# f-dangel/vivit

Hardware: AMD Instinct MI355X
Metric: GGN eigenpairs/sec (Gram build + symeig), MLP 784-512-10, batch=4096 (higher is better)
Workload: dtype f32

## Files before the change

### vivit_amd/csrc/sy2sb.hip

```cpp
#include <cstdlib>

#include "common.h"
#include "device_utils.h"
#include "eig_internal.h"

namespace vivit {

constexpr int SNB = 64;
constexpr int QT = 128;
constexpr int SGRP = 8;

__global__ __launch_bounds__(256) void sb_panel_load_kernel(const float *__restrict__ A, int64_t lda, int64_t j0, int64_t mp,
                                                            float *__restrict__ pan) {
  const int64_t idx = (int64_t)blockIdx.x * 256 + threadIdx.x;
  if (idx >= mp * SNB) return;
  const int64_t r = idx / SNB, c = idx - r * SNB;
  pan[idx] = A[(j0 + SNB + r) * lda + j0 + c];
}

__global__ __launch_bounds__(256) void sb_panel_load_row_kernel(const float *__restrict__ A, int64_t lda, int64_t j0, int64_t mp,
                                                                float *__restrict__ pan) {
  __shared__ float t[SNB][SNB + 1];
  const int64_t r0 = (int64_t)blockIdx.x * SNB;
  const int tid = threadIdx.x;
  for (int idx = tid; idx < SNB * SNB; idx += 256) {
    const int c = idx / SNB, rr = idx % SNB;
    t[c][rr] = r0 + rr < mp ? A[(j0 + c) * lda + j0 + SNB + r0 + rr] : 0.f;
  }
  __syncthreads();
  for (int idx = tid; idx < SNB * SNB; idx += 256) {
    const int rr = idx / SNB, c = idx % SNB;
    if (r0 + rr < mp) pan[(r0 + rr) * SNB + c] = t[c][rr];
  }
}

__global__ __launch_bounds__(256) void coef_gather_kernel(const float *__restrict__ S, int64_t lds_, int64_t g, int kp,
                                                          float *__restrict__ Coef) {
  const int idx = blockIdx.x * 256 + threadIdx.x;
  if (idx >= SNB * kp) return;
  const int k = idx / SNB, m = idx % SNB;
  Coef[(int64_t)m * kp + k] = S[(int64_t)k * lds_ + g + m];
}


__global__ __launch_bounds__(256) void qr_step_kernel(float *__restrict__ pan, int64_t mp, int c, int ncol, int nwg, QrPart pt,
                                                      float *__restrict__ vdst1, float *__restrict__ vdst2, int64_t lds_, int64_t gi0,
                                                      float *__restrict__ A, int64_t lda, int64_t j0,
                                                      float *__restrict__ tau1, float *__restrict__ betas) {
  __shared__ float tile[QT][SNB + 1];
  __shared__ float vs[QT], xs2[QT];
  __shared__ float zs[SNB];
  __shared__ float zq[4][SNB];
  __shared__ __attribute__((aligned(16))) float zq16[16][SNB];
  const int tid = threadIdx.x;
  const int64_t r0 = (int64_t)blockIdx.x * QT;
  constexpr int NTL = QT * (SNB / 4) / 256;
  float4 tl[NTL];
#pragma unroll
  for (int i = 0; i < NTL; ++i) {
    const int idx = tid + 256 * i;
    const int rl = idx / (SNB / 4), c4 = (idx - rl * (SNB / 4)) * 4;
    const int64_t r = r0 + rl;
    tl[i] = *reinterpret_cast<const float4 *>(pan + (r < mp ? r : 0) * SNB + c4);
  }
  const int par = c & 1;
  const float *uin = pt.u + (int64_t)par * nwg * SNB;
  const float *din = pt.diag + par * SNB;
  const int cq4 = tid & 15, q16 = tid >> 4;
  float4 pv[20];
#pragma unroll
  for (int i = 0; i < 20; ++i) {
    const int w = q16 + 16 * i;
    pv[i] = *reinterpret_cast<const float4 *>(uin + (int64_t)(w < nwg ? w : 0) * SNB + 4 * cq4);
  }
  const float din_c = din[c >= 0 ? c : 0], din_t = din[tid & (SNB - 1)];
  __builtin_amdgcn_sched_barrier(0);
#pragma unroll
  for (int i = 0; i < NTL; ++i) {
    const int idx = tid + 256 * i;
    const int rl = idx / (SNB / 4), c4 = (idx - rl * (SNB / 4)) * 4;
    const bool ok = r0 + rl < mp;
    tile[rl][c4 + 0] = ok ? tl[i].x : 0.f;
    tile[rl][c4 + 1] = ok ? tl[i].y : 0.f;
    tile[rl][c4 + 2] = ok ? tl[i].z : 0.f;
    tile[rl][c4 + 3] = ok ? tl[i].w : 0.f;
  }
  if (c >= 0) {
    {
      float4 acc = make_float4(0.f, 0.f, 0.f, 0.f);
#pragma unroll
      for (int i = 0; i < 20; ++i)
        if (q16 + 16 * i < nwg) { acc.x += pv[i].x; acc.y += pv[i].y; acc.z += pv[i].z; acc.w += pv[i].w; }
      for (int w0 = q16 + 16 * 20; w0 < nwg; w0 += 16 * 20) {
        float4 v[20];
#pragma unroll
        for (int i = 0; i < 20; ++i) {
          const int w = w0 + 16 * i;
          v[i] = *reinterpret_cast<const float4 *>(uin + (int64_t)(w < nwg ? w : 0) * SNB + 4 * cq4);
        }
#pragma unroll
        for (int i = 0; i < 20; ++i)
          if (w0 + 16 * i < nwg) { acc.x += v[i].x; acc.y += v[i].y; acc.z += v[i].z; acc.w += v[i].w; }
      }
      *reinterpret_cast<float4 *>(&zq16[q16][4 * cq4]) = acc;
    }
    __syncthreads();
    float ssq = 0.f;
#pragma unroll
    for (int g2 = 0; g2 < 16; ++g2) ssq += zq16[g2][c];
    const float alpha = din_c;
    float tau = 0.f, beta = alpha, scal = 0.f;
    if (ssq > 0.f) {
      beta = -copysignf(sqrt_nr(alpha * alpha + ssq), alpha);
      tau = (beta - alpha) * rcp_nr(beta);
      scal = rcp_nr(alpha - beta);
    }
    if (tid < SNB) {
      float u = 0.f;
#pragma unroll
      for (int g2 = 0; g2 < 16; ++g2) u += zq16[g2][tid];
      zs[tid] = tid > c ? tau * (din_t + scal * u) : 0.f;
    }
    if (tid < QT) {
      const int64_t r = r0 + tid;
      float v = 0.f;
      if (r < mp) {
        if (r == c) v = 1.f;
        else if (r > c) v = tile[tid][c] * scal;
        vdst1[(int64_t)c * lds_ + gi0 + r] = v;
        vdst2[(int64_t)c * lds_ + gi0 + r] = v;
        if (r >= c) A[(j0 + c) * lda + gi0 + r] = v;
      }
      vs[tid] = v;
    }
    if (blockIdx.x == 0 && tid == 0) { tau1[j0 + c] = tau; betas[c] = beta; }
  } else {
    if (tid < QT) vs[tid] = 0.f;
    if (tid < SNB) zs[tid] = 0.f;
  }
  __syncthreads();
  const int cn = c + 1;
  const bool has_next = cn < ncol;
  if (tid < QT) {
    const int64_t r = r0 + tid;
    xs2[tid] = (has_next && r > cn && r < mp) ? tile[tid][cn] - vs[tid] * zs[cn] : 0.f;
  }
  __syncthreads();
  {
    const int cc = tid & 63, q = tid >> 6;
    const float zc = zs[cc];
    float acc = 0.f;
#pragma unroll 8
    for (int i = 0; i < QT / 4; ++i) {
      const int rl = q + 4 * i;
      const float v = vs[rl];
      float x = tile[rl][cc];
      if (cc > c && v != 0.f) {
        x -= v * zc;
        tile[rl][cc] = x;
        if (r0 + rl < mp) pan[(r0 + rl) * SNB + cc] = x;
      }
      acc += xs2[rl] * x;
    }
    zq[q][cc] = acc;
  }
  if (!has_next) return;
  __syncthreads();
  {
    const int par = cn & 1;
    if (tid < SNB) pt.u[((int64_t)par * nwg + blockIdx.x) * SNB + tid] = (zq[0][tid] + zq[1][tid]) + (zq[2][tid] + zq[3][tid]);
    if (cn >= r0 && cn < r0 + QT && tid < SNB) pt.diag[par * SNB + tid] = tile[cn - r0][tid];
  }
}

constexpr int QP_WG = 32, QP_THREADS = 512;
struct QrPersistWs {
  float *ubuf;
  float *dbuf;
  int *counter;
  int *tmo;
  int attempt;
  int fault;
};

__device__ __forceinline__ float sel8(float a0, float a1, float a2, float a3, float a4, float a5, float a6, float a7, int j) {
  const float t0 = (j & 1) ? a1 : a0, t1 = (j & 1) ? a3 : a2, t2 = (j & 1) ? a5 : a4, t3 = (j & 1) ? a7 : a6;
  const float u0 = (j & 2) ? t1 : t0, u1 = (j & 2) ? t3 : t2;
  return (j & 4) ? u1 : u0;
}

template <int RI>
__global__ __launch_bounds__(QP_THREADS) void qr_persist_kernel(float *__restrict__ pan, int64_t mp, int ncol, QrPersistWs pw,
                                                                float *__restrict__ vdst1, float *__restrict__ vdst2, int64_t lds_,
                                                                int64_t gi0, float *__restrict__ A, int64_t lda, int64_t j0,
                                                                float *__restrict__ tau1, float *__restrict__ betas) {
  if ((blockIdx.x & 7) != 0) return;
  if (pw.attempt == 1 && __hip_atomic_load(pw.counter + 1, __ATOMIC_RELAXED, __HIP_MEMORY_SCOPE_AGENT) != PERSIST_ABORT) return;
  int *const cnt = pw.counter + 8 * pw.attempt;
  const int w = blockIdx.x >> 3;
  const int tid = threadIdx.x, lane = tid & 63, wave = tid >> 6;
  const int cg = tid & 7, rs = tid >> 3;
  constexpr int RW = 64 * RI;
  const int64_t rbase = (int64_t)w * RW;
  __shared__ float s_u[SNB], s_d[SNB], s_dn[SNB];
  __shared__ float s_red[QP_THREADS / 64][SNB];
  __shared__ float s_v[RW];
  __shared__ int s_flag[2];

  float x[RI][8];
#pragma unroll
  for (int i = 0; i < RI; ++i) {
    const int64_t r = rbase + rs + 64 * i;
    const float *src = pan + (r < mp ? r : 0) * SNB + 8 * cg;
    const float4 a = *reinterpret_cast<const float4 *>(src), b = *reinterpret_cast<const float4 *>(src + 4);
    const bool ok = r < mp;
    x[i][0] = ok ? a.x : 0.f; x[i][1] = ok ? a.y : 0.f; x[i][2] = ok ? a.z : 0.f; x[i][3] = ok ? a.w : 0.f;
    x[i][4] = ok ? b.x : 0.f; x[i][5] = ok ? b.y : 0.f; x[i][6] = ok ? b.z : 0.f; x[i][7] = ok ? b.w : 0.f;
  }
  if (tid == 0) {
    int xcc;
    __asm__ volatile("s_getreg_b32 %0, hwreg(HW_REG_XCC_ID)" : "=s"(xcc));
    __hip_atomic_store(pw.counter + 32 + w, xcc & 15, __ATOMIC_RELAXED, __HIP_MEMORY_SCOPE_AGENT);
    __asm__ volatile("s_waitcnt vmcnt(0)" ::: "memory");
    const bool go = persist_arrive(cnt, cnt + 1, QP_WG, ((pw.fault >> pw.attempt) & 1) ? 0ull : PERSIST_TIMEOUT_TICKS);
    const int dead = go ? 0 : 2;
    int slow = 0;
    const int x0 = __hip_atomic_load(pw.counter + 32, __ATOMIC_RELAXED, __HIP_MEMORY_SCOPE_AGENT);
    for (int i = 1; i < QP_WG; ++i) slow |= __hip_atomic_load(pw.counter + 32 + i, __ATOMIC_RELAXED, __HIP_MEMORY_SCOPE_AGENT) != x0;
    s_flag[0] = slow;
    s_flag[1] = dead;
  }
  __syncthreads();
  const bool slow = s_flag[0] != 0;
  if (s_flag[1] == 2) {
    if (tid == 0 && w == 0 && pw.attempt == 1) {
      __hip_atomic_fetch_or(pw.tmo, PERSIST_TMO_PANEL_QR, __ATOMIC_RELAXED, __HIP_MEMORY_SCOPE_AGENT);
      betas[0] = __builtin_nanf("");
    }
    return;
  }
  const int grp = lane & ~7;

  auto publish = [&](int cn) __attribute__((always_inline)) {
    float acc[8];
#pragma unroll
    for (int j = 0; j < 8; ++j) acc[j] = 0.f;
#pragma unroll
    for (int i = 0; i < RI; ++i) {
      const int64_t r = rbase + rs + 64 * i;
      float xn = __shfl(sel8(x[i][0], x[i][1], x[i][2], x[i][3], x[i][4], x[i][5], x[i][6], x[i][7], cn & 7), grp | (cn >> 3), 64);
      xn = (r > cn && r < mp) ? xn : 0.f;
#pragma unroll
      for (int j = 0; j < 8; ++j) acc[j] = fmaf(xn, x[i][j], acc[j]);
    }
#pragma unroll
    for (int j = 0; j < 8; ++j) {
      acc[j] += __shfl_xor(acc[j], 8, 64);
      acc[j] += __shfl_xor(acc[j], 16, 64);
      acc[j] += __shfl_xor(acc[j], 32, 64);
    }
    if (lane < 8) {
#pragma unroll
      for (int j = 0; j < 8; ++j) s_red[wave][8 * lane + j] = acc[j];
    }
    if (w == 0 && rs == cn) {
#pragma unroll
      for (int j = 0; j < 8; ++j) s_dn[8 * cg + j] = x[0][j];
    }
  };
  auto send = [&](int par) __attribute__((always_inline)) {
    if (wave == 0) {
      float u = 0.f;
#pragma unroll
      for (int q = 0; q < QP_THREADS / 64; ++q) u += s_red[q][lane];
      float *ub = pw.ubuf + ((size_t)par * QP_WG + w) * SNB + lane, *db = pw.dbuf + (size_t)par * SNB + lane;
      if (slow) {
        __hip_atomic_store(ub, u, __ATOMIC_RELAXED, __HIP_MEMORY_SCOPE_AGENT);
        if (w == 0) __hip_atomic_store(db, s_dn[lane], __ATOMIC_RELAXED, __HIP_MEMORY_SCOPE_AGENT);
      } else {
        *ub = u;
        if (w == 0) *db = s_dn[lane];
      }
      __asm__ volatile("s_waitcnt vmcnt(0)" ::: "memory");
      if (lane == 0) __hip_atomic_fetch_add(cnt, 1, __ATOMIC_RELAXED, __HIP_MEMORY_SCOPE_AGENT);
    }
  };

  publish(0);
  __syncthreads();
  send(0);
  for (int c = 0; c < ncol && !s_flag[1]; ++c) {
    const int par = c & 1;
    if (wave == 0) {
      const int target = (c + 2) * QP_WG;
      const unsigned long long t0 = __builtin_amdgcn_s_memrealtime();
      while (__hip_atomic_load(cnt, __ATOMIC_RELAXED, __HIP_MEMORY_SCOPE_AGENT) < target)
        if (__builtin_amdgcn_s_memrealtime() - t0 > PERSIST_TIMEOUT_TICKS) { s_flag[1] = 1; break; }
      const float *ub = pw.ubuf + (size_t)par * QP_WG * SNB + lane;
      float pv[QP_WG];
#pragma unroll
      for (int q = 0; q < QP_WG; ++q) pv[q] = __hip_atomic_load(ub + q * SNB, __ATOMIC_RELAXED, __HIP_MEMORY_SCOPE_AGENT);
      const float dn = __hip_atomic_load(pw.dbuf + (size_t)par * SNB + lane, __ATOMIC_RELAXED, __HIP_MEMORY_SCOPE_AGENT);
      float u = 0.f;
#pragma unroll
      for (int q = 0; q < QP_WG; ++q) u += pv[q];
      s_u[lane] = u;
      s_d[lane] = dn;
    }
    __syncthreads();
    if (s_flag[1]) break;
    const float ssq = s_u[c], alpha = s_d[c];
    float tau = 0.f, beta = alpha, scal = 0.f;
    if (ssq > 0.f) {
      beta = -copysignf(sqrt_nr(alpha * alpha + ssq), alpha);
      tau = (beta - alpha) * rcp_nr(beta);
      scal = rcp_nr(alpha - beta);
    }
    float z[8];
#pragma unroll
    for (int j = 0; j < 8; ++j) {
      const int cc = 8 * cg + j;
      z[j] = cc > c ? tau * (s_d[cc] + scal * s_u[cc]) : 0.f;
    }
#pragma unroll
    for (int i = 0; i < RI; ++i) {
      const int64_t r = rbase + rs + 64 * i;
      const float xc = __shfl(sel8(x[i][0], x[i][1], x[i][2], x[i][3], x[i][4], x[i][5], x[i][6], x[i][7], c & 7), grp | (c >> 3), 64);
      const float v = r == c ? 1.f : ((r > c && r < mp) ? xc * scal : 0.f);
      if (cg == 0) s_v[rs + 64 * i] = v;
#pragma unroll
      for (int j = 0; j < 8; ++j) x[i][j] = fmaf(-v, z[j], x[i][j]);
    }
    if (w == 0 && tid == 0) { tau1[j0 + c] = tau; betas[c] = beta; }
    const bool has_next = c + 1 < ncol;
    if (has_next) publish(c + 1);
    __syncthreads();
    if (has_next) send(par ^ 1);
    for (int idx = tid; idx < RW; idx += QP_THREADS) {
      const int64_t r = rbase + idx;
      if (r < mp) {
        const float v = s_v[idx];
        vdst1[(int64_t)c * lds_ + gi0 + r] = v;
        vdst2[(int64_t)c * lds_ + gi0 + r] = v;
        if (r >= c) A[(j0 + c) * lda + gi0 + r] = v;
      }
    }
  }
  if (w == 0) {
    const int64_t r = rs;
    if (r < mp) {
      float *dst = pan + r * SNB + 8 * cg;
      *reinterpret_cast<float4 *>(dst) = make_float4(x[0][0], x[0][1], x[0][2], x[0][3]);
      *reinterpret_cast<float4 *>(dst + 4) = make_float4(x[0][4], x[0][5], x[0][6], x[0][7]);
    }
    if (tid == 0 && s_flag[1]) {
      betas[0] = __builtin_nanf("");
      __hip_atomic_fetch_or(pw.tmo, PERSIST_TMO_PANEL_QR, __ATOMIC_RELAXED, __HIP_MEMORY_SCOPE_AGENT);
    }
  }
}

static bool qr_persist_enabled() {
  static int on = -1;
  if (on < 0) {
    const char *e = getenv("VIVIT_QR_PERSIST");
    on = e ? atoi(e) : 1;
  }
  return on != 0 && persist_override() != 0;
}
constexpr size_t QR_PERSIST_WS_BYTES = sizeof(float) * (2 * QP_WG * SNB + 2 * SNB) + 64 * sizeof(int) + 256;

static bool qr_persist_launch(float *pan, int64_t mp, int ncol, void *wsp, float *v1, float *v2, int64_t ldn, int64_t gi0, float *A,
                              int64_t lda, int64_t j0, float *tau1, float *betas, hipStream_t stream) {
  if (!qr_persist_enabled() || mp > (int64_t)QP_WG * 64 * 20 || device_cu_count() < 256) return false;
  QrPersistWs pw;
  pw.ubuf = reinterpret_cast<float *>(align_up(reinterpret_cast<uintptr_t>(wsp), 256));
  pw.dbuf = pw.ubuf + 2 * QP_WG * SNB;
  pw.counter = reinterpret_cast<int *>(pw.dbuf + 2 * SNB);
  pw.tmo = persist_timeout_word(stream);
  pw.fault = persist_fault();
  if (!pw.tmo) return false;
  if (hipMemsetAsync(pw.counter, 0, 64 * sizeof(int), stream) != hipSuccess) return false;
  const int64_t ri = cdiv(mp, (int64_t)QP_WG * 64);
  const dim3 grid(8 * QP_WG);
#define QP_LAUNCH(RI) qr_persist_kernel<RI><<<grid, QP_THREADS, 0, stream>>>(pan, mp, ncol, pw, v1, v2, ldn, gi0, A, lda, j0, tau1, betas)
  for (int attempt = 0; attempt < 2; ++attempt) {
    pw.attempt = attempt;
    if (ri <= 1) QP_LAUNCH(1);
    else if (ri <= 2) QP_LAUNCH(2);
    else if (ri <= 3) QP_LAUNCH(3);
    else if (ri <= 5) QP_LAUNCH(5);
    else if (ri <= 8) QP_LAUNCH(8);
    else if (ri <= 12) QP_LAUNCH(12);
    else if (ri <= 16) QP_LAUNCH(16);
    else QP_LAUNCH(20);
  }
#undef QP_LAUNCH
  return true;
}

struct Sk64Args {
  const float *Coef;
  const float *B;
  float *Out;
  int64_t ldcoef, ldb, ldo, N;
  int K;
  float alpha, beta;
};
constexpr int SK_LDC = 36, SK_COLS = 128, SK_LDB = SK_COLS + 4, SK_NT = SK_COLS / 64;

__global__ __launch_bounds__(256) void skinny64_kernel(Sk64Args p) {
  __shared__ __attribute__((aligned(16))) float sC[64 * SK_LDC];
  __shared__ __attribute__((aligned(16))) float sB[32 * SK_LDB];
  const int tid = threadIdx.x, lane = tid & 63, wave = tid >> 6;
  const int r = lane & 31, h = lane >> 5, wm = wave >> 1, wn = wave & 1;
  const int64_t c0 = (int64_t)blockIdx.x * SK_COLS;
  f32x16 acc[SK_NT];
#pragma unroll
  for (int t = 0; t < SK_NT; ++t)
#pragma unroll
    for (int e = 0; e < 16; ++e) acc[t][e] = 0.f;
  constexpr int NLB = 32 * SK_COLS / 4 / 256;
  float4 rc[2], rb[NLB];
  auto gload = [&](int k0) __attribute__((always_inline)) {
#pragma unroll
    for (int i = 0; i < 2; ++i) {
      const int idx = tid + 256 * i;
      const int m = idx >> 3, kq = (idx & 7) * 4;
      rc[i] = *reinterpret_cast<const float4 *>(p.Coef + (int64_t)m * p.ldcoef + k0 + kq);
    }
#pragma unroll
    for (int i = 0; i < NLB; ++i) {
      const int idx = tid + 256 * i;
      const int kr = idx / (SK_COLS / 4), cq = (idx % (SK_COLS / 4)) * 4;
      const int64_t c = c0 + cq;
      rb[i] = *reinterpret_cast<const float4 *>(p.B + (int64_t)(k0 + kr) * p.ldb + (c < p.N ? c : 0));
    }
    __builtin_amdgcn_sched_barrier(0);
  };
  gload(0);
  for (int k0 = 0; k0 < p.K; k0 += 32) {
    __syncthreads();
#pragma unroll
    for (int i = 0; i < 2; ++i) {
      const int idx = tid + 256 * i;
      *reinterpret_cast<float4 *>(sC + (idx >> 3) * SK_LDC + (idx & 7) * 4) = rc[i];
    }
#pragma unroll
    for (int i = 0; i < NLB; ++i) {
      const int idx = tid + 256 * i;
      const int kr = idx / (SK_COLS / 4), cq = (idx % (SK_COLS / 4)) * 4;
      *reinterpret_cast<float4 *>(sB + kr * SK_LDB + cq) = c0 + cq < p.N ? rb[i] : make_float4(0.f, 0.f, 0.f, 0.f);
    }
    __syncthreads();
    if (k0 + 32 < p.K) gload(k0 + 32);
    const float *pa = sC + (32 * wm + r) * SK_LDC + 4 * h;
#pragma unroll
    for (int j = 0; j < 4; ++j) {
      const float4 a4 = *reinterpret_cast<const float4 *>(pa + 8 * j);
      const float av[4] = {a4.x, a4.y, a4.z, a4.w};
      float bv[4][SK_NT];
#pragma unroll
      for (int i = 0; i < 4; ++i)
#pragma unroll
        for (int t = 0; t < SK_NT; ++t) bv[i][t] = sB[(8 * j + 4 * h + i) * SK_LDB + 64 * wn + 32 * t + r];
#pragma unroll
      for (int i = 0; i < 4; ++i)
#pragma unroll
        for (int t = 0; t < SK_NT; ++t) acc[t] = __builtin_amdgcn_mfma_f32_32x32x2f32(av[i], bv[i][t], acc[t], 0, 0, 0);
    }
  }
#pragma unroll
  for (int t = 0; t < SK_NT; ++t) {
    const int64_t c = c0 + 64 * wn + 32 * t + r;
    if (c < p.N) {
#pragma unroll
      for (int e = 0; e < 16; ++e) {
        const int m = 32 * wm + (e & 3) + 8 * (e >> 2) + 4 * h;
        float *o = p.Out + (int64_t)m * p.ldo + c;
        float v = p.alpha * acc[t][e];
        if (p.beta != 0.f) v += p.beta * *o;
        *o = v;
      }
    }
  }
}

static bool skinny64_launch(const float *Coef, int64_t ldcoef, const float *B, int64_t ldb, float *Out, int64_t ldo, int64_t N, int64_t K,
                            float alpha, float beta, hipStream_t stream) {
  if (K < 32 || K % 32 != 0 || K > 4096 || N % 4 != 0 || ldb % 4 != 0 || ldcoef % 4 != 0 ||
      (reinterpret_cast<uintptr_t>(Coef) & 15) || (reinterpret_cast<uintptr_t>(B) & 15))
    return false;
  Sk64Args a;
  a.Coef = Coef; a.B = B; a.Out = Out; a.ldcoef = ldcoef; a.ldb = ldb; a.ldo = ldo; a.N = N; a.K = (int)K; a.alpha = alpha; a.beta = beta;
  skinny64_kernel<<<(unsigned)cdiv(N, SK_COLS), 256, 0, stream>>>(a);
  return true;
}

__global__ __launch_bounds__(256) void w_coef_kernel(const float *__restrict__ T, const float *__restrict__ G, float *__restrict__ Coef) {
  __shared__ float sT[SNB][SNB + 1], sG[SNB][SNB + 1], sU[SNB][SNB + 1];
  const int tid = threadIdx.x, lane = tid & 63, wave = tid >> 6;
  const int r = lane & 31, h = lane >> 5, qi = (wave >> 1) * 32, qj = (wave & 1) * 32;
  for (int idx = tid; idx < SNB * SNB; idx += 256) {
    sT[idx / SNB][idx % SNB] = T[idx];
    sG[idx / SNB][idx % SNB] = G[idx];
  }
  __syncthreads();
  f32x16 acc;
#pragma unroll
  for (int e = 0; e < 16; ++e) acc[e] = 0.f;
#pragma unroll 8
  for (int s2 = 0; s2 < SNB / 2; ++s2) acc = __builtin_amdgcn_mfma_f32_32x32x2f32(sT[2 * s2 + h][qi + r], sG[2 * s2 + h][qj + r], acc, 0, 0, 0);
#pragma unroll
  for (int e = 0; e < 16; ++e) sU[qi + (e & 3) + 8 * (e >> 2) + 4 * h][qj + r] = acc[e];
  __syncthreads();
#pragma unroll
  for (int e = 0; e < 16; ++e) acc[e] = 0.f;
#pragma unroll 8
  for (int s2 = 0; s2 < SNB / 2; ++s2) acc = __builtin_amdgcn_mfma_f32_32x32x2f32(sU[qi + r][2 * s2 + h], sT[2 * s2 + h][qj + r], acc, 0, 0, 0);
#pragma unroll
  for (int e = 0; e < 16; ++e) {
    const int a_ = qi + (e & 3) + 8 * (e >> 2) + 4 * h, b_ = qj + r;
    Coef[a_ * 2 * SNB + b_] = -0.5f * acc[e];
    Coef[a_ * 2 * SNB + SNB + b_] = sT[b_][a_];
  }
}

__global__ __launch_bounds__(256) void sb_panel_store_kernel(float *__restrict__ A, int64_t lda, int64_t j0, int64_t mp,
                                                             const float *__restrict__ pan, const float *__restrict__ betas) {
  const int idx = blockIdx.x * 256 + threadIdx.x;
  if (idx >= SNB * SNB) return;
  const int r = idx / SNB, c = idx - r * SNB;
  if (r >= mp) return;
  A[(j0 + SNB + r) * lda + j0 + c] = (r < c) ? pan[(int64_t)r * SNB + c] : (r == c ? betas[c] : 0.f);
}

__global__ __launch_bounds__(256) void larft_kernel(const float *__restrict__ S, int64_t lds_, const float *__restrict__ tau, int nb,
                                                    int nvalid, float *__restrict__ T) {
  constexpr int H = SNB / 2, LD = SNB + 1;
  __shared__ float Ss[SNB * LD], Ts[SNB * LD], Xs[H * (H + 1)], taus[SNB];
  const int tid = threadIdx.x;
  for (int idx = tid; idx < SNB * SNB; idx += 256) {
    Ss[(idx / SNB) * LD + (idx % SNB)] = S[(int64_t)(idx / SNB) * lds_ + (idx % SNB)];
    Ts[(idx / SNB) * LD + (idx % SNB)] = 0.f;
  }
  if (tid < SNB) taus[tid] = (tid < nvalid && tid < nb) ? tau[tid] : 0.f;
  __syncthreads();
  if (tid < SNB) {
    const int half = tid / H, j = tid % H;
    const float *Sb = Ss + half * (H * LD + H), *tb = taus + half * H;
    float t[H];
#pragma unroll
    for (int c = 0; c < H; ++c) t[c] = 0.f;
#pragma unroll
    for (int i = H - 1; i >= 0; --i) {
      float acc = 0.f;
#pragma unroll
      for (int c = i + 1; c < H; ++c) acc += Sb[i * LD + c] * t[c];
      t[i] = i == j ? tb[j] : (i < j ? -tb[i] * acc : 0.f);
    }
    float *Tb = Ts + half * (H * LD + H);
#pragma unroll
    for (int i = 0; i < H; ++i) Tb[i * LD + j] = t[i];
  }
  __syncthreads();
  if (tid < 64) {
    const int r = tid & 31, h = tid >> 5;
    f32x16 acc;
#pragma unroll
    for (int e = 0; e < 16; ++e) acc[e] = 0.f;
#pragma unroll 8
    for (int s2 = 0; s2 < H / 2; ++s2)
      acc = __builtin_amdgcn_mfma_f32_32x32x2f32(Ss[r * LD + H + 2 * s2 + h], Ts[(H + 2 * s2 + h) * LD + H + r], acc, 0, 0, 0);
#pragma unroll
    for (int e = 0; e < 16; ++e) Xs[((e & 3) + 8 * (e >> 2) + 4 * h) * (H + 1) + r] = acc[e];
  }
  __syncthreads();
  if (tid < 64) {
    const int r = tid & 31, h = tid >> 5;
    f32x16 acc;
#pragma unroll
    for (int e = 0; e < 16; ++e) acc[e] = 0.f;
#pragma unroll 8
    for (int s2 = 0; s2 < H / 2; ++s2)
      acc = __builtin_amdgcn_mfma_f32_32x32x2f32(Ts[r * LD + 2 * s2 + h], Xs[(2 * s2 + h) * (H + 1) + r], acc, 0, 0, 0);
#pragma unroll
    for (int e = 0; e < 16; ++e) Ts[((e & 3) + 8 * (e >> 2) + 4 * h) * LD + H + r] = -acc[e];
  }
  __syncthreads();
  for (int idx = tid; idx < SNB * SNB; idx += 256) T[idx] = Ts[(idx / SNB) * LD + (idx % SNB)];
}

__global__ __launch_bounds__(256) void sb_extract_band_kernel(const float *__restrict__ A, int64_t lda, int64_t n,
                                                              float *__restrict__ AB, int64_t ldab) {
  const int64_t idx = (int64_t)blockIdx.x * 256 + threadIdx.x;
  if (idx >= n * ldab) return;
  const int64_t i = idx / ldab;
  const int d = (int)(idx - i * ldab);
  const int64_t j = i - 2 * SNB + d;
  AB[idx] = (d >= SNB && d <= 2 * SNB && j >= 0) ? A[i * lda + j] : 0.f;
}

static size_t sy2sb_gemm_ws_bytes(int64_t n) {
  size_t m = 0;
  for (int64_t mp = 1; mp <= n; mp = mp < 4096 ? mp * 2 : mp + 4096) {
    const int64_t q = mp < n ? mp : n;
    size_t a = gemm_workspace_bytes(SNB, SNB, q, false);
    size_t b = gemm_workspace_bytes(SNB, q, q, false);
    size_t c = gemm_workspace_bytes(SNB, q, SNB, false);
    size_t d = 0, e = 0, f = 0;
    for (int g = 1; g < SGRP; ++g) {
      const size_t d1 = gemm_workspace_bytes(SNB, 2 * SNB * g + SNB, q, false), e1 = gemm_workspace_bytes(SNB, q, 2 * SNB * g, false);
      const size_t f1 = gemm_workspace_bytes(q, SNB, 2 * SNB * g, false);
      d = d1 > d ? d1 : d; e = e1 > e ? e1 : e; f = f1 > f ? f1 : f;
    }
    m = a > m ? a : m; m = b > m ? b : m; m = c > m ? c : m;
    m = d > m ? d : m; m = e > m ? e : m; m = f > m ? f : m;
    const size_t u = gemm_workspace_bytes(q, q, (int64_t)2 * SNB * SGRP, true);
    m = u > m ? u : m;
  }
  size_t a = gemm_workspace_bytes(SNB, SNB, n, false), b = gemm_workspace_bytes(SNB, n, n, false);
  m = a > m ? a : m; m = b > m ? b : m;
  return m * 2;
}

Sy2sbWs sy2sb_layout(Arena &a, int64_t n) {
  const int64_t nwg = cdiv(n, QT) + 1;
  Sy2sbWs ws;
  ws.pan = a.take<float>(n * SNB);
  ws.stackA = a.take<float>(2 * SGRP * SNB * n);
  ws.stackB = a.take<float>(2 * SGRP * SNB * n);
  ws.xt = a.take<float>(SNB * n);
  ws.G12 = a.take<float>(SNB * 2 * SNB * SGRP);
  ws.qp.u = a.take<float>(2 * nwg * SNB);
  ws.qp.diag = a.take<float>(2 * SNB);
  ws.qpw = a.take<char>(QR_PERSIST_WS_BYTES);
  ws.S = a.take<float>(SNB * SNB);
  ws.T = a.take<float>(SNB * SNB);
  ws.Y3 = a.take<float>(SNB * SNB);
  ws.S2 = a.take<float>(SNB * SNB);
  ws.tau1 = a.take<float>(n);
  ws.betas = a.take<float>(SNB);
  ws.gws_bytes = sy2sb_gemm_ws_bytes(n);
  ws.gws = a.take<char>(ws.gws_bytes);
  return ws;
}

size_t sy2sb_workspace_bytes(int64_t n) {
  Arena m;
  sy2sb_layout(m, n);
  return m.used() + 1024;
}

int sy2sb_launch(float *A, int64_t n, int64_t lda, const Sy2sbWs &ws, hipStream_t stream) {
  if (hipMemsetAsync(ws.tau1, 0, sizeof(float) * n, stream) != hipSuccess) return VIVIT_E_LAUNCH;

  const int64_t ldn = n;
  const bool rowmode = (n % 4 == 0) && (lda % 4 == 0) && (reinterpret_cast<uintptr_t>(A) & 15) == 0;
  auto factor_panel = [&](int64_t j0, float *v1, float *v2) -> int {
    const int64_t mp = n - j0 - SNB, gi0 = j0 + SNB;
    const int ncol = (int)(mp < SNB ? mp : SNB);
    const int g = (int)cdiv(mp, QT);
    if (rowmode) sb_panel_load_row_kernel<<<(unsigned)cdiv(mp, SNB), 256, 0, stream>>>(A, lda, j0, mp, ws.pan);
    else sb_panel_load_kernel<<<(unsigned)cdiv(mp * SNB, 256), 256, 0, stream>>>(A, lda, j0, mp, ws.pan);
    if (!qr_persist_launch(ws.pan, mp, ncol, ws.qpw, v1, v2, ldn, gi0, A, lda, j0, ws.tau1, ws.betas, stream))
      for (int c = -1; c < ncol; ++c)
        qr_step_kernel<<<g, 256, 0, stream>>>(ws.pan, mp, c, ncol, g, ws.qp, v1, v2, ldn, gi0, A, lda, j0, ws.tau1, ws.betas);
    sb_panel_store_kernel<<<(unsigned)cdiv(SNB * SNB, 256), 256, 0, stream>>>(A, lda, j0, mp, ws.pan, ws.betas);
    return launch_status();
  };
  auto compute_w = [&](int64_t j0, float *Vt, float *Wt, float *Wcopy, int64_t kp, const float *sAg, const float *sBg) -> int {
    const int64_t mp = n - j0 - SNB, gi0 = j0 + SNB;
    const int ncol = (int)(mp < SNB ? mp : SNB);
    float *A22 = A + gi0 * lda + gi0;
    int st;
    prof_mark(PROF_STAGE_SY2SB, stream);
    st = gemm_launch(LAY_K, LAY_M, Vt, A22, Wt, SNB, mp, mp, ldn, lda, ldn, 1.f, 0.f, false, ws.gws, ws.gws_bytes, stream);
    prof_mark(PROF_STAGE_SY2SB_PP, stream);
    if (st != VIVIT_OK) return st;
    const int64_t ldg = kp + SNB;
    st = gemm_launch(LAY_K, LAY_K, Vt, sAg, ws.G12, SNB, ldg, mp, ldn, ldn, ldg, 1.f, 0.f, false, ws.gws, ws.gws_bytes, stream);
    if (st != VIVIT_OK) return st;
    larft_kernel<<<1, 256, 0, stream>>>(ws.G12 + kp, ldg, ws.tau1 + j0, SNB, ncol, ws.T);
    if (kp > 0) {
      if (!skinny64_launch(ws.G12, ldg, sBg, ldn, Wt, ldn, mp, kp, -1.f, 1.f, stream)) {
        st = gemm_launch(LAY_K, LAY_M, ws.G12, sBg, Wt, SNB, mp, kp, ldg, ldn, ldn, -1.f, 1.f, false, ws.gws, ws.gws_bytes, stream);
        if (st != VIVIT_OK) return st;
      }
    }
    st = gemm_launch(LAY_K, LAY_K, Wt, Vt, ws.S2, SNB, SNB, mp, ldn, ldn, SNB, 1.f, 0.f, false, ws.gws, ws.gws_bytes, stream);
    if (st != VIVIT_OK) return st;
    w_coef_kernel<<<1, 256, 0, stream>>>(ws.T, ws.S2, ws.G12);
    if (Wt == Vt + (int64_t)SNB * ldn &&
        skinny64_launch(ws.G12, 2 * SNB, Vt, ldn, Wcopy, ldn, mp, 2 * SNB, 1.f, 0.f, stream))
      return hipMemcpy2DAsync(Wt, sizeof(float) * ldn, Wcopy, sizeof(float) * ldn, sizeof(float) * mp, SNB, hipMemcpyDeviceToDevice,
                              stream) == hipSuccess ? VIVIT_OK : VIVIT_E_LAUNCH;
    float *Xt = ws.xt + gi0;
    st = gemm_launch(LAY_M, LAY_M, ws.T, Wt, Xt, SNB, mp, SNB, SNB, ldn, ldn, 1.f, 0.f, false, ws.gws, ws.gws_bytes, stream);
    if (st != VIVIT_OK) return st;
    if (hipMemcpy2DAsync(Wt, sizeof(float) * ldn, Xt, sizeof(float) * ldn, sizeof(float) * mp, SNB, hipMemcpyDeviceToDevice,
                         stream) != hipSuccess)
      return VIVIT_E_LAUNCH;
    st = gemm_launch(LAY_K, LAY_M, ws.G12, Vt, Wt, SNB, mp, SNB, 2 * SNB, ldn, ldn, 1.f, 1.f, false, ws.gws, ws.gws_bytes, stream);
    if (st != VIVIT_OK) return st;
    return hipMemcpy2DAsync(Wcopy, sizeof(float) * ldn, Wt, sizeof(float) * ldn, sizeof(float) * mp, SNB, hipMemcpyDeviceToDevice,
                            stream) == hipSuccess ? VIVIT_OK : VIVIT_E_LAUNCH;
  };

  float *sA = ws.stackA, *sB = ws.stackB;
  for (int64_t j0 = 0; j0 + SNB < n;) {
    int st;
    if (hipMemsetAsync(sA, 0, sizeof(float) * 2 * SGRP * SNB * n, stream) != hipSuccess) return VIVIT_E_LAUNCH;
    if (hipMemsetAsync(sB, 0, sizeof(float) * 2 * SGRP * SNB * n, stream) != hipSuccess) return VIVIT_E_LAUNCH;
    int np = 0;
    int64_t gi_last = 0;
    for (; np < SGRP && j0 + SNB < n; ++np, j0 += SNB) {
      const int64_t gi = j0 + SNB;
      const int64_t kp = (int64_t)2 * SNB * np;
      if (np > 0) {
        const int64_t gc = gi - SNB;
        bool done = false;
        if (rowmode) {
          coef_gather_kernel<<<(unsigned)cdiv(SNB * kp, 256), 256, 0, stream>>>(sA, ldn, gc, (int)kp, ws.G12);
          done = skinny64_launch(ws.G12, kp, sB + gc, ldn, A + gc * lda + gc, lda, n - gc, kp, -1.f, 1.f, stream);
        }
        if (!done) {
          if (rowmode) return VIVIT_E_UNSUPPORTED;
          st = gemm_launch(LAY_M, LAY_M, sA + gc, sB + gc, A + gc * lda + gc, n - gc, SNB, kp, ldn, ldn, lda, -1.f, 1.f, false,
                           ws.gws, ws.gws_bytes, stream);
          if (st != VIVIT_OK) return st;
        }
      }
      float *Vrow = sA + kp * n, *Wrow = sA + (kp + SNB) * n;
      st = factor_panel(j0, Vrow, sB + (kp + SNB) * n);
      if (st != VIVIT_OK) return st;
      st = compute_w(j0, Vrow + gi, Wrow + gi, sB + kp * n + gi, kp, sA + gi, sB + gi);
      if (st != VIVIT_OK) return st;
      gi_last = gi;
    }
    const int64_t mt = n - gi_last;
    prof_mark(PROF_STAGE_SY2SB, stream);
    st = gemm_launch(LAY_M, LAY_M, sA + gi_last, sB + gi_last, A + gi_last * lda + gi_last, mt, mt, (int64_t)2 * SNB * np, ldn, ldn,
                     lda, -1.f, 1.f, true, ws.gws, ws.gws_bytes, stream);
    prof_mark(PROF_STAGE_SY2SB_UPD, stream);
    if (st != VIVIT_OK) return st;
  }
  return launch_status();
}

struct PanelQrWs {
  QrPart qp;
  float *S;
  void *qpw, *gws;
  size_t gws_bytes;
};

static PanelQrWs panel_qr_layout(Arena &a, int64_t mp) {
  const int64_t nwg = cdiv(mp, QT) + 1;
  PanelQrWs ws;
  ws.qp.u = a.take<float>(2 * nwg * SNB);
  ws.qp.diag = a.take<float>(2 * SNB);
  ws.S = a.take<float>(SNB * SNB);
  ws.qpw = a.take<char>(QR_PERSIST_WS_BYTES);
  ws.gws_bytes = gemm_workspace_bytes(SNB, SNB, mp, false);
  ws.gws = a.take<char>(ws.gws_bytes);
  return ws;
}

size_t sy2sb_panel_qr_workspace_bytes(int64_t mp) {
  Arena m;
  panel_qr_layout(m, mp);
  return m.used() + 1024;
}

int sy2sb_panel_qr_launch(float *pan, int64_t mp, float *Vt, int64_t ldv, float *tau, float *betas, float *T, void *wsbase,
                          size_t ws_bytes, hipStream_t stream) {
  if (ws_bytes < sy2sb_panel_qr_workspace_bytes(mp)) return VIVIT_E_WORKSPACE;
  Arena a(wsbase, ws_bytes);
  const PanelQrWs ws = panel_qr_layout(a, mp);
  if (a.overflow()) return VIVIT_E_WORKSPACE;
  const QrPart qp = ws.qp;
  float *S = ws.S;
  void *qpw = ws.qpw, *gws = ws.gws;
  const size_t gws_bytes = ws.gws_bytes;
  const int ncol = (int)(mp < SNB ? mp : SNB);
  const int g = (int)cdiv(mp, QT);
  if (hipMemsetAsync(tau, 0, sizeof(float) * SNB, stream) != hipSuccess) return VIVIT_E_LAUNCH;
  if (hipMemsetAsync(betas, 0, sizeof(float) * SNB, stream) != hipSuccess) return VIVIT_E_LAUNCH;
  if (hipMemset2DAsync(Vt, sizeof(float) * ldv, 0, sizeof(float) * mp, SNB, stream) != hipSuccess) return VIVIT_E_LAUNCH;
  if (!qr_persist_launch(pan, mp, ncol, qpw, Vt, Vt, ldv, 0, Vt, ldv, 0, tau, betas, stream))
    for (int c = -1; c < ncol; ++c)
      qr_step_kernel<<<g, 256, 0, stream>>>(pan, mp, c, ncol, g, qp, Vt, Vt, ldv, 0, Vt, ldv, 0, tau, betas);
  int st = gemm_launch(LAY_K, LAY_K, Vt, Vt, S, SNB, SNB, mp, ldv, ldv, SNB, 1.f, 0.f, false, gws, gws_bytes, stream);
  if (st != VIVIT_OK) return st;
  larft_kernel<<<1, 256, 0, stream>>>(S, SNB, tau, SNB, ncol, T);
  return launch_status();
}

int sy2sb_extract_band_launch(const float *A, int64_t lda, int64_t n, float *AB, int64_t ldab, hipStream_t stream) {
  sb_extract_band_kernel<<<(unsigned)cdiv(n * ldab, 256), 256, 0, stream>>>(A, lda, n, AB, ldab);
  return launch_status();
}

}

using namespace vivit;

extern "C" {

size_t vivit_sy2sb_f32_workspace_bytes(int64_t n) { return n > 0 ? sy2sb_workspace_bytes(n) : 0; }

int vivit_sy2sb_f32(float *A, int64_t n, int64_t lda, float *AB, float *tau1, void *workspace, size_t workspace_bytes,
                    void *stream) {
  if (n < 1 || !A || !AB || !tau1 || lda < n) return VIVIT_E_BADARG;
  if (!workspace || workspace_bytes < sy2sb_workspace_bytes(n)) return VIVIT_E_WORKSPACE;
  hipStream_t s = static_cast<hipStream_t>(stream);
  Arena a(workspace, workspace_bytes);
  const Sy2sbWs ws = sy2sb_layout(a, n);
  if (a.overflow()) return VIVIT_E_WORKSPACE;
  int st = sy2sb_launch(A, n, lda, ws, s);
  if (st != VIVIT_OK) return st;
  st = sy2sb_extract_band_launch(A, lda, n, AB, 2 * SNB + 1, s);
  if (st != VIVIT_OK) return st;
  if (hipMemcpyAsync(tau1, ws.tau1, sizeof(float) * n, hipMemcpyDeviceToDevice, s) != hipSuccess) return VIVIT_E_LAUNCH;
  return VIVIT_OK;
}

size_t vivit_sy2sb_panel_qr_f32_workspace_bytes(int64_t mp) { return mp > 0 ? sy2sb_panel_qr_workspace_bytes(mp) : 0; }

int vivit_sy2sb_panel_qr_f32(float *pan, int64_t mp, float *Vt, int64_t ldv, float *tau, float *betas, float *T, void *workspace,
                             size_t workspace_bytes, void *stream) {
  if (mp < 1 || !pan || !Vt || !tau || !betas || !T || ldv < mp) return VIVIT_E_BADARG;
  if (!workspace) return VIVIT_E_WORKSPACE;
  return sy2sb_panel_qr_launch(pan, mp, Vt, ldv, tau, betas, T, workspace, workspace_bytes, static_cast<hipStream_t>(stream));
}

}
```

Before: 7602.

## Fuse coef gather and W copy into templated double-buffered skinny64 kernel

Templates the skinny64 MFMA kernel on column width and a gather mode. The gather mode reads the transposed coefficient stack directly, which removes the separate coef_gather kernel. The kernel now double-buffers LDS to overlap global loads with MFMA work and drops one barrier per k-step. It also picks a narrower column tile when the grid would be too small to fill the CUs, and a second output pointer replaces a device-to-device memcpy. The cost is more LDS per block and strided LDS reads of coefficients in gather mode.

```diff
diff --git a/vivit_amd/csrc/sy2sb.hip b/vivit_amd/csrc/sy2sb.hip
--- a/vivit_amd/csrc/sy2sb.hip
+++ b/vivit_amd/csrc/sy2sb.hip
@@ -32,14 +32,6 @@
     const int rr = idx / SNB, c = idx % SNB;
     if (r0 + rr < mp) pan[(r0 + rr) * SNB + c] = t[c][rr];
   }
-}
-
-__global__ __launch_bounds__(256) void coef_gather_kernel(const float *__restrict__ S, int64_t lds_, int64_t g, int kp,
-                                                          float *__restrict__ Coef) {
-  const int idx = blockIdx.x * 256 + threadIdx.x;
-  if (idx >= SNB * kp) return;
-  const int k = idx / SNB, m = idx % SNB;
-  Coef[(int64_t)m * kp + k] = S[(int64_t)k * lds_ + g + m];
 }
 
 
@@ -402,77 +394,103 @@
 struct Sk64Args {
   const float *Coef;
   const float *B;
-  float *Out;
+  float *Out, *Out2;
   int64_t ldcoef, ldb, ldo, N;
   int K;
   float alpha, beta;
 };
-constexpr int SK_LDC = 36, SK_COLS = 128, SK_LDB = SK_COLS + 4, SK_NT = SK_COLS / 64;
-
-__global__ __launch_bounds__(256) void skinny64_kernel(Sk64Args p) {
-  __shared__ __attribute__((aligned(16))) float sC[64 * SK_LDC];
-  __shared__ __attribute__((aligned(16))) float sB[32 * SK_LDB];
+constexpr int SK_LDC = 36, SK_LDCT = SNB + 4, SK_CBUF = 64 * SK_LDC;
+
+template <int COLS, bool GATHER>
+__global__ __launch_bounds__(COLS >= 64 ? 256 : 128) void skinny64_kernel(Sk64Args p) {
+  constexpr int WN = COLS >= 64 ? 2 : 1;
+  constexpr int NT = COLS / (32 * WN);
+  constexpr int NTHR = 128 * WN;
+  constexpr int LDB = COLS + 4;
+  constexpr int NLC = 64 * 32 / 4 / NTHR;
+  constexpr int NLB = 32 * COLS / 4 / NTHR;
+  static_assert(32 * SK_LDCT <= SK_CBUF && NLB >= 1, "tile");
+  __shared__ __attribute__((aligned(16))) float sC[2][SK_CBUF];
+  __shared__ __attribute__((aligned(16))) float sB[2][32 * LDB];
   const int tid = threadIdx.x, lane = tid & 63, wave = tid >> 6;
-  const int r = lane & 31, h = lane >> 5, wm = wave >> 1, wn = wave & 1;
-  const int64_t c0 = (int64_t)blockIdx.x * SK_COLS;
-  f32x16 acc[SK_NT];
-#pragma unroll
-  for (int t = 0; t < SK_NT; ++t)
+  const int r = lane & 31, h = lane >> 5, wm = wave / WN, wn = wave % WN;
+  const int64_t c0 = (int64_t)blockIdx.x * COLS;
+  f32x16 acc[NT];
+#pragma unroll
+  for (int t = 0; t < NT; ++t)
 #pragma unroll
     for (int e = 0; e < 16; ++e) acc[t][e] = 0.f;
-  constexpr int NLB = 32 * SK_COLS / 4 / 256;
-  float4 rc[2], rb[NLB];
+  f32x4 rc[NLC], rb[NLB];
   auto gload = [&](int k0) __attribute__((always_inline)) {
 #pragma unroll
-    for (int i = 0; i < 2; ++i) {
-      const int idx = tid + 256 * i;
-      const int m = idx >> 3, kq = (idx & 7) * 4;
-      rc[i] = *reinterpret_cast<const float4 *>(p.Coef + (int64_t)m * p.ldcoef + k0 + kq);
+    for (int i = 0; i < NLC; ++i) {
+      const int idx = tid + NTHR * i;
+      if (GATHER) {
+        const int kr = idx >> 4, mq = (idx & 15) * 4;
+        rc[i] = *reinterpret_cast<const f32x4 *>(p.Coef + (int64_t)(k0 + kr) * p.ldcoef + mq);
+      } else {
+        const int m = idx >> 3, kq = (idx & 7) * 4;
+        rc[i] = *reinterpret_cast<const f32x4 *>(p.Coef + (int64_t)m * p.ldcoef + k0 + kq);
+      }
     }
 #pragma unroll
     for (int i = 0; i < NLB; ++i) {
-      const int idx = tid + 256 * i;
-      const int kr = idx / (SK_COLS / 4), cq = (idx % (SK_COLS / 4)) * 4;
+      const int idx = tid + NTHR * i;
+      const int kr = idx / (COLS / 4), cq = (idx % (COLS / 4)) * 4;
       const int64_t c = c0 + cq;
-      rb[i] = *reinterpret_cast<const float4 *>(p.B + (int64_t)(k0 + kr) * p.ldb + (c < p.N ? c : 0));
+      rb[i] = *reinterpret_cast<const f32x4 *>(p.B + (int64_t)(k0 + kr) * p.ldb + (c < p.N ? c : c0));
     }
     __builtin_amdgcn_sched_barrier(0);
   };
+  auto lstore = [&](int buf) __attribute__((always_inline)) {
+#pragma unroll
+    for (int i = 0; i < NLC; ++i) {
+      const int idx = tid + NTHR * i;
+      if (GATHER) *reinterpret_cast<f32x4 *>(sC[buf] + (idx >> 4) * SK_LDCT + (idx & 15) * 4) = rc[i];
+      else *reinterpret_cast<f32x4 *>(sC[buf] + (idx >> 3) * SK_LDC + (idx & 7) * 4) = rc[i];
+    }
+#pragma unroll
+    for (int i = 0; i < NLB; ++i) {
+      const int idx = tid + NTHR * i;
+      const int kr = idx / (COLS / 4), cq = (idx % (COLS / 4)) * 4;
+      *reinterpret_cast<f32x4 *>(sB[buf] + kr * LDB + cq) = c0 + cq < p.N ? rb[i] : f32x4{0.f, 0.f, 0.f, 0.f};
+    }
+  };
   gload(0);
-  for (int k0 = 0; k0 < p.K; k0 += 32) {
+  lstore(0);
+  if (32 < p.K) gload(32);
+  int cur = 0;
+  for (int k0 = 0; k0 < p.K; k0 += 32, cur ^= 1) {
     __syncthreads();
-#pragma unroll
-    for (int i = 0; i < 2; ++i) {
-      const int idx = tid + 256 * i;
-      *reinterpret_cast<float4 *>(sC + (idx >> 3) * SK_LDC + (idx & 7) * 4) = rc[i];
-    }
-#pragma unroll
-    for (int i = 0; i < NLB; ++i) {
-      const int idx = tid + 256 * i;
-      const int kr = idx / (SK_COLS / 4), cq = (idx % (SK_COLS / 4)) * 4;
-      *reinterpret_cast<float4 *>(sB + kr * SK_LDB + cq) = c0 + cq < p.N ? rb[i] : make_float4(0.f, 0.f, 0.f, 0.f);
-    }
-    __syncthreads();
-    if (k0 + 32 < p.K) gload(k0 + 32);
-    const float *pa = sC + (32 * wm + r) * SK_LDC + 4 * h;
+    if (k0 + 32 < p.K) {
+      lstore(cur ^ 1);
+      if (k0 + 64 < p.K) gload(k0 + 64);
+    }
+    const float *cb = sC[cur], *bb = sB[cur];
 #pragma unroll
     for (int j = 0; j < 4; ++j) {
-      const float4 a4 = *reinterpret_cast<const float4 *>(pa + 8 * j);
-      const float av[4] = {a4.x, a4.y, a4.z, a4.w};
-      float bv[4][SK_NT];
+      float av[4];
+      if (GATHER) {
+#pragma unroll
+        for (int i = 0; i < 4; ++i) av[i] = cb[(8 * j + 4 * h + i) * SK_LDCT + 32 * wm + r];
+      } else {
+        const f32x4 a4 = *reinterpret_cast<const f32x4 *>(cb + (32 * wm + r) * SK_LDC + 4 * h + 8 * j);
+        av[0] = a4[0]; av[1] = a4[1]; av[2] = a4[2]; av[3] = a4[3];
+      }
+      float bv[4][NT];
 #pragma unroll
       for (int i = 0; i < 4; ++i)
 #pragma unroll
-        for (int t = 0; t < SK_NT; ++t) bv[i][t] = sB[(8 * j + 4 * h + i) * SK_LDB + 64 * wn + 32 * t + r];
+        for (int t = 0; t < NT; ++t) bv[i][t] = bb[(8 * j + 4 * h + i) * LDB + 32 * NT * wn + 32 * t + r];
 #pragma unroll
       for (int i = 0; i < 4; ++i)
 #pragma unroll
-        for (int t = 0; t < SK_NT; ++t) acc[t] = __builtin_amdgcn_mfma_f32_32x32x2f32(av[i], bv[i][t], acc[t], 0, 0, 0);
-    }
-  }
-#pragma unroll
-  for (int t = 0; t < SK_NT; ++t) {
-    const int64_t c = c0 + 64 * wn + 32 * t + r;
+        for (int t = 0; t < NT; ++t) acc[t] = __builtin_amdgcn_mfma_f32_32x32x2f32(av[i], bv[i][t], acc[t], 0, 0, 0);
+    }
+  }
+#pragma unroll
+  for (int t = 0; t < NT; ++t) {
+    const int64_t c = c0 + 32 * NT * wn + 32 * t + r;
     if (c < p.N) {
 #pragma unroll
       for (int e = 0; e < 16; ++e) {
@@ -481,19 +499,29 @@
         float v = p.alpha * acc[t][e];
         if (p.beta != 0.f) v += p.beta * *o;
         *o = v;
-      }
-    }
-  }
-}
-
-static bool skinny64_launch(const float *Coef, int64_t ldcoef, const float *B, int64_t ldb, float *Out, int64_t ldo, int64_t N, int64_t K,
-                            float alpha, float beta, hipStream_t stream) {
+        if (p.Out2) p.Out2[(int64_t)m * p.ldo + c] = v;
+      }
+    }
+  }
+}
+
+static bool skinny64_launch(const float *Coef, int64_t ldcoef, bool gather, const float *B, int64_t ldb, float *Out, float *Out2,
+                            int64_t ldo, int64_t N, int64_t K, float alpha, float beta, hipStream_t stream) {
   if (K < 32 || K % 32 != 0 || K > 4096 || N % 4 != 0 || ldb % 4 != 0 || ldcoef % 4 != 0 ||
       (reinterpret_cast<uintptr_t>(Coef) & 15) || (reinterpret_cast<uintptr_t>(B) & 15))
     return false;
   Sk64Args a;
-  a.Coef = Coef; a.B = B; a.Out = Out; a.ldcoef = ldcoef; a.ldb = ldb; a.ldo = ldo; a.N = N; a.K = (int)K; a.alpha = alpha; a.beta = beta;
-  skinny64_kernel<<<(unsigned)cdiv(N, SK_COLS), 256, 0, stream>>>(a);
+  a.Coef = Coef; a.B = B; a.Out = Out; a.Out2 = Out2; a.ldcoef = ldcoef; a.ldb = ldb; a.ldo = ldo; a.N = N; a.K = (int)K;
+  a.alpha = alpha; a.beta = beta;
+  const int cus = device_cu_count() > 0 ? device_cu_count() : 256;
+  const int cols = cdiv(N, (int64_t)128) >= 2 * cus ? 128 : (cdiv(N, (int64_t)64) >= 2 * cus ? 64 : 32);
+#define SK_LAUNCH(COLS, G) skinny64_kernel<COLS, G><<<(unsigned)cdiv(N, (int64_t)COLS), COLS >= 64 ? 256 : 128, 0, stream>>>(a)
+  if (gather) {
+    if (cols == 128) SK_LAUNCH(128, true); else if (cols == 64) SK_LAUNCH(64, true); else SK_LAUNCH(32, true);
+  } else {
+    if (cols == 128) SK_LAUNCH(128, false); else if (cols == 64) SK_LAUNCH(64, false); else SK_LAUNCH(32, false);
+  }
+#undef SK_LAUNCH
   return true;
 }
 
@@ -683,7 +711,7 @@
     if (st != VIVIT_OK) return st;
     larft_kernel<<<1, 256, 0, stream>>>(ws.G12 + kp, ldg, ws.tau1 + j0, SNB, ncol, ws.T);
     if (kp > 0) {
-      if (!skinny64_launch(ws.G12, ldg, sBg, ldn, Wt, ldn, mp, kp, -1.f, 1.f, stream)) {
+      if (!skinny64_launch(ws.G12, ldg, false, sBg, ldn, Wt, nullptr, ldn, mp, kp, -1.f, 1.f, stream)) {
         st = gemm_launch(LAY_K, LAY_M, ws.G12, sBg, Wt, SNB, mp, kp, ldg, ldn, ldn, -1.f, 1.f, false, ws.gws, ws.gws_bytes, stream);
         if (st != VIVIT_OK) return st;
       }
@@ -692,9 +720,8 @@
     if (st != VIVIT_OK) return st;
     w_coef_kernel<<<1, 256, 0, stream>>>(ws.T, ws.S2, ws.G12);
     if (Wt == Vt + (int64_t)SNB * ldn &&
-        skinny64_launch(ws.G12, 2 * SNB, Vt, ldn, Wcopy, ldn, mp, 2 * SNB, 1.f, 0.f, stream))
-      return hipMemcpy2DAsync(Wt, sizeof(float) * ldn, Wcopy, sizeof(float) * ldn, sizeof(float) * mp, SNB, hipMemcpyDeviceToDevice,
-                              stream) == hipSuccess ? VIVIT_OK : VIVIT_E_LAUNCH;
+        skinny64_launch(ws.G12, 2 * SNB, false, Vt, ldn, Wcopy, Wt, ldn, mp, 2 * SNB, 1.f, 0.f, stream))
+      return launch_status();
     float *Xt = ws.xt + gi0;
     st = gemm_launch(LAY_M, LAY_M, ws.T, Wt, Xt, SNB, mp, SNB, SNB, ldn, ldn, 1.f, 0.f, false, ws.gws, ws.gws_bytes, stream);
     if (st != VIVIT_OK) return st;
@@ -721,8 +748,7 @@
         const int64_t gc = gi - SNB;
         bool done = false;
         if (rowmode) {
-          coef_gather_kernel<<<(unsigned)cdiv(SNB * kp, 256), 256, 0, stream>>>(sA, ldn, gc, (int)kp, ws.G12);
-          done = skinny64_launch(ws.G12, kp, sB + gc, ldn, A + gc * lda + gc, lda, n - gc, kp, -1.f, 1.f, stream);
+          done = skinny64_launch(sA + gc, ldn, true, sB + gc, ldn, A + gc * lda + gc, nullptr, lda, n - gc, kp, -1.f, 1.f, stream);
         }
         if (!done) {
           if (rowmode) return VIVIT_E_UNSUPPORTED;
```

New measurement: 7653 (median of 4 runs). No clear change (+0.7%).
